# xenji/kafka-topic-analyzer

Measured on AMD Instinct MI355X. Metric: records/sec whole-node + achieved HBM GB/s, 256-part 256B-mean synthetic topic, higher is better.
Workload: dtype u64; 1 GPU; c4: 256-partition synthetic topic, mixed key/value sizes (mean record ~256 B), partitions sharded p % n_gpus; records_per_gpu=1073741824, partitions=256, partition_order=random, bytes_per_record=20, parallelism=partition-sharded x1, forced_collectives=False, exchange=none (1 GPU)

## Files before the change

### kafka_topic_analyzer_amd/csrc/kta_kernels.hip

```cpp
#include "kta_kernels.h"

#include <limits.h>
#include <type_traits>

namespace kta {


constexpr uint32_t kCntBits = 21;
constexpr uint64_t kCntMask = (1ull << kCntBits) - 1;
constexpr uint32_t kFlushTiles = 256;
#ifndef KTA_SCAN_PREFETCH
#define KTA_SCAN_PREFETCH 1
#endif
#ifndef KTA_PACKED_LOADS_ONLY
#define KTA_PACKED_LOADS_ONLY 0
#endif
constexpr int kTilePrefetch = KTA_SCAN_PREFETCH;
static_assert(kTilePrefetch == 1 || kTilePrefetch == 2, "the prefetch ring has two or three slots");
#ifndef KTA_PACKED_PREFETCH
#define KTA_PACKED_PREFETCH 1
#endif
constexpr int kPackedPrefetch = KTA_PACKED_PREFETCH;
static_assert(kPackedPrefetch == 1 || kPackedPrefetch == 2, "the prefetch ring has two or three slots");

struct Quad {
    int4 p, k, v;
    longlong2 t0, t1;
    long long base;
    uint32_t compact;
};
constexpr uint32_t kQuadCompact = 1u, kQuadLens16 = 2u, kQuadSummed = 4u;

typedef int v4i __attribute__((ext_vector_type(4)));
typedef int v2i __attribute__((ext_vector_type(2)));
typedef long long v2l __attribute__((ext_vector_type(2)));
static_assert(KTA_TILE_RECORDS == 4u * kWG, "a layout tile is one scan tile: 256 lanes x 4 records");

template <bool NT>
__device__ __forceinline__ void load_quad(Quad &q, const ScanColumns &c, uint64_t qi)
{
    if (NT) {
        const v4i p = __builtin_nontemporal_load(reinterpret_cast<const v4i *>(c.partition) + qi);
        const v4i k = __builtin_nontemporal_load(reinterpret_cast<const v4i *>(c.key_len) + qi);
        const v4i v = __builtin_nontemporal_load(reinterpret_cast<const v4i *>(c.val_len) + qi);
        const v2l t0 = __builtin_nontemporal_load(reinterpret_cast<const v2l *>(c.ts_ms) + 2 * qi);
        const v2l t1 = __builtin_nontemporal_load(reinterpret_cast<const v2l *>(c.ts_ms) + 2 * qi + 1);
        q.p = make_int4(p.x, p.y, p.z, p.w);
        q.k = make_int4(k.x, k.y, k.z, k.w);
        q.v = make_int4(v.x, v.y, v.z, v.w);
        q.t0 = make_longlong2(t0.x, t0.y);
        q.t1 = make_longlong2(t1.x, t1.y);
    } else {
        q.p = reinterpret_cast<const int4 *>(c.partition)[qi];
        q.k = reinterpret_cast<const int4 *>(c.key_len)[qi];
        q.v = reinterpret_cast<const int4 *>(c.val_len)[qi];
        q.t0 = reinterpret_cast<const longlong2 *>(c.ts_ms)[2 * qi];
        q.t1 = reinterpret_cast<const longlong2 *>(c.ts_ms)[2 * qi + 1];
    }
    q.compact = 0u;
}

template <bool NT>
__device__ __forceinline__ int4 load16(const void *col, uint64_t i)
{
    if (NT) {
        const v4i x = __builtin_nontemporal_load(reinterpret_cast<const v4i *>(col) + i);
        return make_int4(x.x, x.y, x.z, x.w);
    }
    return reinterpret_cast<const int4 *>(col)[i];
}

__device__ __forceinline__ void tile_sum_extrema(const kta_tile_hdr &h, const kta_tile_sum &s, long long &lo, long long &hi)
{
    const bool timed = (s.flags & KTA_TILE_SUM_TIMED) != 0, untimed = (s.flags & KTA_TILE_SUM_UNTIMED) != 0;
    lo = timed ? (long long)h.ts_base : LLONG_MAX;
    hi = timed ? (long long)((uint64_t)h.ts_base + s.ts_span) : LLONG_MIN;
    lo = (untimed && 0ll < lo) ? 0ll : lo;
    hi = (untimed && 0ll > hi) ? 0ll : hi;
}
__device__ __forceinline__ bool tile_summed(const kta_tile_hdr &h, const kta_tile_sum &s, uint64_t T, const ScanColumns &c, uint64_t n,
                                            uint32_t pc, long long &lo, long long &hi)
{
    const uint64_t first = T * KTA_TILE_RECORDS;
    if (!((s.flags & KTA_TILE_SUM_VALID) && first >= c.rec0 && first + KTA_TILE_RECORDS <= c.rec0 + n && s.part_max < pc)) return false;
    tile_sum_extrema(h, s, lo, hi);
    return true;
}

__device__ __forceinline__ uint32_t quad_valid(uint64_t a, uint64_t n)
{
    uint32_t valid = 0u;
#pragma unroll
    for (uint32_t j = 0; j < 4; j++) valid |= (a + j < n) ? 1u << j : 0u;
    return valid;
}

template <bool NT, bool SUM = false>
__device__ __forceinline__ void load_tile_quad(Quad &q, const ScanColumns &c, uint64_t T, uint32_t tid, uint64_t n = 0, uint32_t pc = 0)
{
    const kta_tile_hdr h = c.hdr[T];
    const kta_tile_sum sm = SUM ? c.sum[T] : kta_tile_sum{0, 0, 0};
    const uint64_t qi = T * (KTA_TILE_RECORDS / 4) + tid;
    const bool lens16 = h.lens == KTA_TILE_LENS_U16;
    q.k = load16<NT>(c.key_len, qi);
    if (!lens16) q.v = load16<NT>(c.val_len, qi);
    if (h.mode != KTA_TILE_COMPACT) {
        q.p = load16<NT>(c.partition, qi);
        const int4 a = load16<NT>(c.ts_ms, 2 * qi), b = load16<NT>(c.ts_ms, 2 * qi + 1);
        q.t0.x = (long long)(((uint64_t)(uint32_t)a.y << 32) | (uint32_t)a.x);
        q.t0.y = (long long)(((uint64_t)(uint32_t)a.w << 32) | (uint32_t)a.z);
        q.t1.x = (long long)(((uint64_t)(uint32_t)b.y << 32) | (uint32_t)b.x);
        q.t1.y = (long long)(((uint64_t)(uint32_t)b.w << 32) | (uint32_t)b.z);
        q.compact = lens16 ? kQuadLens16 : 0u;
        return;
    }
    const uint64_t ci = T * (KTA_TILE_RECORDS / 2) + tid;
    v2i p;
    if (NT) p = __builtin_nontemporal_load(reinterpret_cast<const v2i *>(c.partition) + ci);
    else p = reinterpret_cast<const v2i *>(c.partition)[ci];
    q.p.x = p.x;
    q.p.y = p.y;
    if (SUM) {
        long long lo, hi;
        if (tile_summed(h, sm, T, c, n, pc, lo, hi)) {
            q.t0.x = lo;
            q.t0.y = hi;
            q.compact = kQuadCompact | kQuadSummed | (lens16 ? kQuadLens16 : 0u);
            return;
        }
    }
    const int4 o = load16<NT>(c.ts_ms, ci);
    q.t0.x = (long long)(((uint64_t)(uint32_t)o.y << 32) | (uint32_t)o.x);
    q.t0.y = (long long)(((uint64_t)(uint32_t)o.w << 32) | (uint32_t)o.z);
    q.base = h.ts_base;
    q.compact = kQuadCompact | (lens16 ? kQuadLens16 : 0u);
}

__device__ __forceinline__ void quad_part_ts(const Quad &q, uint32_t (&p)[4], long long (&t)[4])
{
    if (q.compact & kQuadCompact) {
        uint32_t u[4];
        int32_t o[4];
        tile_u16x4((uint32_t)q.p.x, (uint32_t)q.p.y, u);
        tile_i32x4(q.t0.x, q.t0.y, o);
#pragma unroll
        for (int j = 0; j < 4; j++) {
            p[j] = (uint32_t)tile_unpack_part(u[j]);
            t[j] = tile_unpack_ts(o[j], q.base);
        }
    } else {
        p[0] = (uint32_t)q.p.x, p[1] = (uint32_t)q.p.y, p[2] = (uint32_t)q.p.z, p[3] = (uint32_t)q.p.w;
        t[0] = q.t0.x, t[1] = q.t0.y, t[2] = q.t1.x, t[3] = q.t1.y;
    }
// ... 473 lines not shown
constexpr uint32_t kFrontFlushTiles = 32;
constexpr uint64_t kFrontRecords = (uint64_t)kFrontFlushTiles * KTA_TILE_RECORDS;
static_assert(kFrontRecords <= 0xFFFFu, "count, tombstones and null keys of a front interval fit 16 bits");
static_assert(kFrontRecords + (kFrontRecords << 16) <= 0xFFFFFFFFull, "count | tombstones << 16 stays in W1's low dword");
static_assert(kFrontRecords * (KTA_COMPACT_LEN_NONE - 1u) < (1ull << 31), "a front interval's u16 sizes sum below 2^31");
static_assert(kFrontRecords * KTA_PLANE_KEY_NONE < (1ull << 23), "a front interval's raw plane key bytes sum below 2^23");
static_assert(kFrontRecords * KTA_COMPACT_LEN_NONE < (1ull << 31), "a front interval's raw plane value words sum below 2^31");

struct PackedLds {
    unsigned long long *W1, *W2;
    unsigned long long *B;
};

__device__ __forceinline__ unsigned long long pack_dwords(uint32_t lo, uint32_t hi)
{
    return ((unsigned long long)hi << 32) | lo;
}

template <bool LENS16>
__device__ __forceinline__ void packed_quad_lens(const Quad &q, const uint32_t (&pt)[4], const bool (&ok)[4], uint32_t P,
                                                 uint32_t rep_log2, uint32_t rep, const PackedLds &L, LaneState &st)
{
    uint32_t tomb[4], knull[4], ks[4], vs[4];
    if (LENS16) {
        uint32_t ku[4], vu[4];
        tile_u16x4((uint32_t)q.k.x, (uint32_t)q.k.y, ku);
        tile_u16x4((uint32_t)q.k.z, (uint32_t)q.k.w, vu);
#pragma unroll
        for (int j = 0; j < 4; j++) {
            knull[j] = ku[j] == KTA_COMPACT_LEN_NONE;
            tomb[j] = vu[j] == KTA_COMPACT_LEN_NONE;
            ks[j] = knull[j] ? 0u : ku[j];
            vs[j] = tomb[j] ? 0u : vu[j];
        }
    } else {
        const int32_t kl[4] = {q.k.x, q.k.y, q.k.z, q.k.w}, vl[4] = {q.v.x, q.v.y, q.v.z, q.v.w};
#pragma unroll
        for (int j = 0; j < 4; j++) {
            knull[j] = (uint32_t)kl[j] >> 31;
            tomb[j] = (uint32_t)vl[j] >> 31;
            ks[j] = knull[j] ? 0u : (uint32_t)kl[j];
            vs[j] = tomb[j] ? 0u : (uint32_t)vl[j];
        }
    }
#pragma unroll
    for (int j = 0; j < 4; j++) {
        const bool sized = ok[j] && !tomb[j];
        const uint32_t sz = ks[j] + vs[j];
        st.smin = min(st.smin, sized ? sz : 0xFFFFFFFFu);
        st.smax = max(st.smax, sized ? sz : 0u);
    }
#if KTA_PACKED_LOADS_ONLY
    st.bad += pt[0] ^ pt[1] ^ pt[2] ^ pt[3];
    return;
#endif
    const bool uniform = ok[0] && ok[1] && ok[2] && ok[3] && pt[0] == pt[1] && pt[0] == pt[2] && pt[0] == pt[3];
    if (uniform) {
        const uint32_t slot = (pt[0] << rep_log2) | rep;
        const uint32_t tombs = tomb[0] + tomb[1] + tomb[2] + tomb[3];
        const uint32_t knulls = knull[0] + knull[1] + knull[2] + knull[3];
        if (LENS16) {
            atomicAdd(&L.W1[slot], pack_dwords(4u | (tombs << 16), ks[0] + ks[1] + ks[2] + ks[3]));
            atomicAdd(&L.W2[slot], pack_dwords(knulls, vs[0] + vs[1] + vs[2] + vs[3]));
        } else {
            atomicAdd(&L.W1[slot], (unsigned long long)(4u | (tombs << 16)));
            atomicAdd(&L.W2[slot], (unsigned long long)knulls);
            atomicAdd(&L.B[3u * P + pt[0]], (unsigned long long)ks[0] + ks[1] + ks[2] + ks[3]);
            atomicAdd(&L.B[4u * P + pt[0]], (unsigned long long)vs[0] + vs[1] + vs[2] + vs[3]);
        }
        return;
    }
#pragma unroll
    for (int j = 0; j < 4; j++) {
        if (!ok[j]) continue;
        const uint32_t slot = (pt[j] << rep_log2) | rep;
        if (LENS16) {
            atomicAdd(&L.W1[slot], pack_dwords(1u | (tomb[j] << 16), ks[j]));
            atomicAdd(&L.W2[slot], pack_dwords(knull[j], vs[j]));
        } else {
            atomicAdd(&L.W1[slot], (unsigned long long)(1u | (tomb[j] << 16)));
            atomicAdd(&L.W2[slot], (unsigned long long)knull[j]);
            atomicAdd(&L.B[3u * P + pt[j]], (unsigned long long)ks[j]);
            atomicAdd(&L.B[4u * P + pt[j]], (unsigned long long)vs[j]);
        }
    }
}

template <int FORM, bool SUM>
__device__ __forceinline__ void packed_quad(const Quad &q, uint32_t valid, uint32_t P, uint32_t rep_log2, uint32_t rep,
                                            const PackedLds &L, LaneState &st)
{
    const uint32_t form = FORM >= 0 ? (uint32_t)FORM : q.compact;
    uint32_t pt[4];
    bool ok[4];
    if (SUM && (form & kQuadSummed)) {
        tile_u16x4((uint32_t)q.p.x, (uint32_t)q.p.y, pt);
#pragma unroll
        for (int j = 0; j < 4; j++) ok[j] = true;
        st.tmin = q.t0.x < st.tmin ? q.t0.x : st.tmin;
        st.tmax = q.t0.y > st.tmax ? q.t0.y : st.tmax;
    } else if (form & kQuadCompact) {
        static_assert(KTA_COMPACT_TS_NONE == INT32_MIN, "the sentinel is neutral for min as u32 and for max as i32");
        const uint32_t pc = min(P, (uint32_t)KTA_COMPACT_PART_NONE);
        int32_t o[4];
        tile_u16x4((uint32_t)q.p.x, (uint32_t)q.p.y, pt);
        tile_i32x4(q.t0.x, q.t0.y, o);
        uint32_t lo = (uint32_t)KTA_COMPACT_TS_NONE;
        int32_t hi = KTA_COMPACT_TS_NONE;
        bool none = false;
#pragma unroll
        for (int j = 0; j < 4; j++) {
            ok[j] = ((valid >> j) & 1u) && pt[j] < pc;
            const int32_t oj = ok[j] ? o[j] : KTA_COMPACT_TS_NONE;
            lo = min(lo, (uint32_t)oj);
            hi = max(hi, oj);
            none = none || (ok[j] && o[j] == KTA_COMPACT_TS_NONE);
        }
        const bool timed = hi >= 0;
        const long long tlo = (long long)((uint64_t)q.base + lo), thi = (long long)((uint64_t)q.base + (uint32_t)hi);
        st.tmin = (timed && tlo < st.tmin) ? tlo : st.tmin;
        st.tmax = (timed && thi > st.tmax) ? thi : st.tmax;
        st.tmin = (none && 0ll < st.tmin) ? 0ll : st.tmin;
        st.tmax = (none && 0ll > st.tmax) ? 0ll : st.tmax;
    } else {
        const long long ts[4] = {q.t0.x, q.t0.y, q.t1.x, q.t1.y};
        pt[0] = (uint32_t)q.p.x, pt[1] = (uint32_t)q.p.y, pt[2] = (uint32_t)q.p.z, pt[3] = (uint32_t)q.p.w;
#pragma unroll
        for (int j = 0; j < 4; j++) {
            ok[j] = ((valid >> j) & 1u) && pt[j] < P;
            const long long t = (ts[j] == -1ll) ? 0ll : ts[j];
            st.tmin = (ok[j] && t < st.tmin) ? t : st.tmin;
            st.tmax = (ok[j] && t > st.tmax) ? t : st.tmax;
        }
    }
    if (!(SUM && (form & kQuadSummed))) {
#pragma unroll
        for (int j = 0; j < 4; j++) st.bad += (((valid >> j) & 1u) && !ok[j]) ? 1u : 0u;
    }
    if (form & kQuadLens16) packed_quad_lens<true>(q, pt, ok, P, rep_log2, rep, L, st);
    else packed_quad_lens<false>(q, pt, ok, P, rep_log2, rep, L, st);
}

template <bool SUM>
__device__ __forceinline__ void accumulate_packed(const Quad &q, uint32_t valid, uint32_t P, uint32_t rep_log2, uint32_t rep,
                                                  const PackedLds &L, LaneState &st)
{
    constexpr uint32_t both = kQuadCompact | kQuadLens16, summed = both | kQuadSummed;
    if (SUM && q.compact == summed) packed_quad<(int)summed, SUM>(q, valid, P, rep_log2, rep, L, st);
    else if ((q.compact & both) == both) packed_quad<(int)both, SUM>(q, valid, P, rep_log2, rep, L, st);
    else packed_quad<-1, SUM>(q, valid, P, rep_log2, rep, L, st);
}

#ifndef KTA_LEAN_PREFETCH
#define KTA_LEAN_PREFETCH 1
#endif
constexpr int kLeanPrefetch = KTA_LEAN_PREFETCH;
static_assert(kLeanPrefetch >= 1 && kLeanPrefetch <= 3, "the lean ring has two, three or four slots");

struct LeanSlot {
    v2i p;
    int4 k;
};
struct PlaneSlot {
    int4 w;
};
constexpr uint64_t kTileColBytes = (uint64_t)KTA_TILE_RECORDS * 4u;

__device__ __forceinline__ void lean_tile(const kta_tile_hdr &h, const kta_tile_sum &s, uint32_t mark, bool whole, uint32_t pc,
                                          bool &lean, bool &plane)
{
    const bool summed = whole && (s.flags & KTA_TILE_SUM_VALID) && s.part_max < pc && h.mode == KTA_TILE_COMPACT;
    plane = summed && mark == 1u;
    lean = summed && !plane && h.lens == KTA_TILE_LENS_U16;
}

template <bool NT>
__device__ __forceinline__ void lean_load(LeanSlot &s, const ScanColumns &c, uint64_t T, uint32_t off8, uint32_t off16)
{
    const char *pb = reinterpret_cast<const char *>(c.partition) + T * kTileColBytes;
    const char *kb = reinterpret_cast<const char *>(c.key_len) + T * kTileColBytes;
    const v2i *pp = reinterpret_cast<const v2i *>(pb + off8);
    const v4i *kp = reinterpret_cast<const v4i *>(kb + off16);
    s.p = NT ? __builtin_nontemporal_load(pp) : *pp;
    const v4i k = NT ? __builtin_nontemporal_load(kp) : *kp;
    s.k = make_int4(k.x, k.y, k.z, k.w);
}
template <bool NT>
__device__ __forceinline__ void lean_load(PlaneSlot &s, const ScanColumns &c, uint64_t T, uint32_t, uint32_t off16)
{
    const char *tb = reinterpret_cast<const char *>(c.ts_ms) + T * (2u * kTileColBytes) + kTilePlaneOffset;
    const v4i *wp = reinterpret_cast<const v4i *>(tb + off16);
    const v4i w = NT ? __builtin_nontemporal_load(wp) : *wp;
    s.w = make_int4(w.x, w.y, w.z, w.w);
}

__device__ __forceinline__ void lean_quad_add(const uint32_t (&pt)[4], const uint32_t (&ku)[4], const uint32_t (&vu)[4],
                                              const uint32_t (&knull)[4], const uint32_t (&tomb)[4], uint32_t rep_log2, uint32_t rep,
                                              const PackedLds &L, LaneState &st)
{
    uint32_t ks[4], vs[4];
#pragma unroll
    for (int j = 0; j < 4; j++) {
        ks[j] = knull[j] ? 0u : ku[j];
        vs[j] = tomb[j] ? 0u : vu[j];
    }
    uint32_t lo[4], hi[4];
#pragma unroll
    for (int j = 0; j < 4; j++) {
        const uint32_t sz = ks[j] + vs[j];
        lo[j] = tomb[j] ? 0xFFFFFFFFu : sz;
        hi[j] = tomb[j] ? 0u : sz;
    }
    st.smin = min(min(min(lo[0], lo[1]), min(lo[2], lo[3])), st.smin);
    st.smax = max(max(max(hi[0], hi[1]), max(hi[2], hi[3])), st.smax);
#if KTA_PACKED_LOADS_ONLY
    st.bad += pt[0] ^ pt[1] ^ pt[2] ^ pt[3];
    return;
#endif
    if (pt[0] == pt[1] && pt[0] == pt[2] && pt[0] == pt[3]) {
        const uint32_t slot = (pt[0] << rep_log2) | rep;
        const uint32_t tombs = tomb[0] + tomb[1] + tomb[2] + tomb[3];
        const uint32_t knulls = knull[0] + knull[1] + knull[2] + knull[3];
        atomicAdd(&L.W1[slot], pack_dwords(4u | (tombs << 16), ks[0] + ks[1] + ks[2] + ks[3]));
        atomicAdd(&L.W2[slot], pack_dwords(knulls, vs[0] + vs[1] + vs[2] + vs[3]));
        return;
    }
#pragma unroll
    for (int j = 0; j < 4; j++) {
        const uint32_t slot = (pt[j] << rep_log2) | rep;
        atomicAdd(&L.W1[slot], pack_dwords(1u | (tomb[j] << 16), ks[j]));
        atomicAdd(&L.W2[slot], pack_dwords(knull[j], vs[j]));
    }
}
__device__ __forceinline__ void lean_quad(const LeanSlot &s, uint32_t rep_log2, uint32_t rep, const PackedLds &L, LaneState &st)
{
    uint32_t pt[4], ku[4], vu[4], tomb[4], knull[4];
    tile_u16x4((uint32_t)s.p.x, (uint32_t)s.p.y, pt);
    tile_u16x4((uint32_t)s.k.x, (uint32_t)s.k.y, ku);
    tile_u16x4((uint32_t)s.k.z, (uint32_t)s.k.w, vu);
#pragma unroll
    for (int j = 0; j < 4; j++) {
        knull[j] = ku[j] == KTA_COMPACT_LEN_NONE;
        tomb[j] = vu[j] == KTA_COMPACT_LEN_NONE;
    }
    lean_quad_add(pt, ku, vu, knull, tomb, rep_log2, rep, L, st);
}
__device__ __forceinline__ void lean_quad(const PlaneSlot &s, uint32_t rep_log2, uint32_t rep, const PackedLds &L, LaneState &st)
{
    const uint32_t w[4] = {(uint32_t)s.w.x, (uint32_t)s.w.y, (uint32_t)s.w.z, (uint32_t)s.w.w};
#if KTA_PACKED_LOADS_ONLY
    st.bad += w[0] ^ w[1] ^ w[2] ^ w[3];
    return;
#endif
    uint32_t pt[4], ku[4], vu[4], tomb[4], knull[4];
#pragma unroll
    for (int j = 0; j < 4; j++) {
        pt[j] = w[j] & 0xFFu;
        ku[j] = (w[j] >> 8) & 0xFFu;
        vu[j] = w[j] >> 16;
        knull[j] = ku[j] == KTA_PLANE_KEY_NONE;
        tomb[j] = vu[j] == KTA_COMPACT_LEN_NONE;
    }
    if (pt[0] == pt[1] && pt[0] == pt[2] && pt[0] == pt[3]) {
        const uint32_t slot = (pt[0] << rep_log2) | rep;
        const uint32_t tombs = tomb[0] + tomb[1] + tomb[2] + tomb[3];
        const uint32_t knulls = knull[0] + knull[1] + knull[2] + knull[3];
        atomicAdd(&L.W1[slot], pack_dwords(4u | (tombs << 16), ku[0] + ku[1] + ku[2] + ku[3]));
        atomicAdd(&L.W2[slot], pack_dwords(knulls, vu[0] + vu[1] + vu[2] + vu[3]));
        return;
    }
#pragma unroll
    for (int j = 0; j < 4; j++) {
        const uint32_t slot = (pt[j] << rep_log2) | rep;
        atomicAdd(&L.W1[slot], pack_dwords(1u | (tomb[j] << 16), ku[j]));
        atomicAdd(&L.W2[slot], pack_dwords(knull[j], vu[j]));
    }
}

struct PackedWg {
    PackedLds L;
    uint32_t P, rep_log2, rep, tid;
    LaneState st;

    __device__ __forceinline__ PackedWg(unsigned long long *lds, uint32_t P_, uint32_t rep_log2_) : P(P_), rep_log2(rep_log2_)
    {
        tid = threadIdx.x;
        const uint32_t slots = P << rep_log2;
        L = PackedLds{lds, lds + slots, lds + 2 * slots};
        for (uint32_t i = tid; i < 2 * slots + kScanCols * P; i += kWG) lds[i] = 0ull;
        __syncthreads();
        rep = tid & ((1u << rep_log2) - 1u);
    }
    __device__ __forceinline__ void front_flush(bool raw = false) const
    {
        const unsigned long long key_none = raw ? KTA_PLANE_KEY_NONE : 0u, val_none = raw ? KTA_COMPACT_LEN_NONE : 0u;
        __syncthreads();
        for (uint32_t p = tid; p < P; p += kWG) {
            unsigned long long w1 = 0, w2 = 0;
            for (uint32_t r = 0; r < (1u << rep_log2); r++) {
                const uint32_t s = (p << rep_log2) | r;
                w1 += L.W1[s];
                w2 += L.W2[s];
                L.W1[s] = 0ull;
                L.W2[s] = 0ull;
            }
            L.B[p] += w1 & 0xFFFFull;
            L.B[P + p] += (w1 >> 16) & 0xFFFFull;
            L.B[2u * P + p] += w2 & 0xFFFFFFFFull;
            L.B[3u * P + p] += (w1 >> 32) - key_none * (w2 & 0xFFFFFFFFull);
            L.B[4u * P + p] += (w2 >> 32) - val_none * ((w1 >> 16) & 0xFFFFull);
        }
        __syncthreads();
    }
    template <bool MERGE = false>
    __device__ __forceinline__ void write_row(uint64_t *row, long long (&s_red)[kWG / 64][6]) const
    {
        for (uint32_t p = tid; p < P; p += kWG)
#pragma unroll
            for (uint32_t j = 0; j < kScanCols; j++) {
                uint64_t &o = row[(uint64_t)p * kScanCols + j];
                if (MERGE) o += L.B[j * P + p];
                else o = L.B[j * P + p];
            }
        write_scan_globals<MERGE>(st, s_red, row, P, tid);
    }
};

constexpr uint32_t kLeanListed = 4;
constexpr uint32_t kScanListA = 5, kScanHandover = 6, kScanListB = 7;
__device__ __forceinline__ uint32_t lean_list_entry(uint64_t list_a, uint64_t list_b, uint32_t i)
{
    return (uint32_t)((i < 2 ? list_a : list_b) >> (32u * (i & 1u)));
}

struct LeanRun {
    uint32_t tile = 0;
    uint32_t step = 0;
    uint32_t end = 0;
    uint32_t whole_lo = 0, whole_hi = 0;
    uint32_t listed = 0;
    uint64_t list_a = 0, list_b = 0;
    uint32_t handover = 0;
    uint32_t since_flush = 0;
};

template <bool NT, bool PLANE>
__device__ __forceinline__ void lean_run(PackedWg &wg, LeanRun &r, const ScanColumns &c, uint64_t t0, uint32_t last, uint32_t pc,
                                         uint32_t rep_log2)
{
    using Slot = typename std::conditional<PLANE, PlaneSlot, LeanSlot>::type;
    const uint32_t tid = wg.tid;
    const uint32_t G = gridDim.x;
    uint32_t stop = r.end;
    bool switched = false;
    uint32_t issued = r.tile;
    uint32_t istep = r.step;
    uint32_t sw_step = 0;
    kta_tile_hdr ah;
    uint2 as;
    uint32_t am = 0;
    auto look_ahead = [&]() {
        const uint64_t T = t0 + (issued < last ? issued : last);
        ah = c.hdr[T], as = reinterpret_cast<const uint2 *>(c.sum)[T];
        if (c.mark) am = c.mark[T];
    };
    auto issue = [&](Slot &s, bool &v) {
        const uint64_t T = t0 + (issued < last ? issued : last);
        const bool in = issued < stop;
        const kta_tile_sum sm{as.x, (uint16_t)(as.y & 0xFFFFu), (uint16_t)(as.y >> 16)};
        bool lean, plane;
        lean_tile(ah, sm, am, issued >= r.whole_lo && issued < r.whole_hi, pc, lean, plane);
        v = (PLANE ? plane : lean) && in;
        const bool other = (PLANE ? lean : plane) && in;
        lean_load<NT>(s, c, T, 8u * tid, 16u * tid);
        if (other) {
            switched = true;
            sw_step = istep;
            stop = issued;
        } else if (in && !v) {
            if (r.listed == kLeanListed) {
                r.handover = istep + 1u;
                r.end = stop = issued;
            } else {
                const uint64_t e = (uint64_t)(istep + 1u) << (32u * (r.listed & 1u));
                if (r.listed < 2) r.list_a |= e;
                else r.list_b |= e;
                r.listed++;
            }
        }
        issued += G;
        istep++;
        look_ahead();
    };
    auto take = [&](const Slot &s, bool v) {
        if (v) {
            lean_quad(s, rep_log2, wg.rep, wg.L, wg.st);
            if (++r.since_flush == kFrontFlushTiles) {
                wg.front_flush(PLANE);
                r.since_flush = 0;
            }
        }
        r.tile += G;
    };
    Slot s0, s1, s2, s3;
    bool v0 = false, v1 = false, v2 = false, v3 = false;
    look_ahead();
    issue(s0, v0);
    if (kLeanPrefetch >= 2) issue(s1, v1);
    if (kLeanPrefetch == 3) issue(s2, v2);
    while (r.tile < stop) {
        if (kLeanPrefetch == 3) {
            issue(s3, v3);
            take(s0, v0);
            issue(s0, v0);
            take(s1, v1);
            issue(s1, v1);
            take(s2, v2);
            issue(s2, v2);
            take(s3, v3);
        } else if (kLeanPrefetch == 2) {
            issue(s2, v2);
            take(s0, v0);
            issue(s0, v0);
            take(s1, v1);
            issue(s1, v1);
            take(s2, v2);
        } else {
            issue(s1, v1);
            take(s0, v0);
            issue(s0, v0);
            take(s1, v1);
        }
    }
    r.step = istep - (uint32_t)kLeanPrefetch;
    if (switched) r.tile = blockIdx.x + sw_step * G, r.step = sw_step;
}

template <bool NT>
__device__ __forceinline__ void packed_scan_lean(const ScanColumns &c, uint64_t n, uint32_t P, uint32_t rep_log2,
                                                 uint64_t *__restrict__ partials, uint32_t row_len, unsigned long long *lds,
                                                 long long (&s_red)[kWG / 64][6])
{
    PackedWg wg(lds, P, rep_log2);
    const uint32_t tid = wg.tid;
    const uint64_t t0 = c.rec0 / KTA_TILE_RECORDS;
    const uint64_t ntiles = (c.rec0 + n + KTA_TILE_RECORDS - 1) / KTA_TILE_RECORDS - t0;
    const uint32_t pc = min(P, (uint32_t)KTA_COMPACT_PART_NONE);
    LeanRun r;
    r.tile = blockIdx.x;
    r.end = (uint32_t)ntiles;
    r.whole_lo = c.rec0 % KTA_TILE_RECORDS ? 1u : 0u;
    r.whole_hi = (uint32_t)((c.rec0 + n) / KTA_TILE_RECORDS - t0);
    const uint32_t last = r.end - 1u;
    bool plane = c.mark != nullptr;
    while (r.tile < r.end) {
        if (plane) lean_run<NT, true>(wg, r, c, t0, last, pc, rep_log2);
        else lean_run<NT, false>(wg, r, c, t0, last, pc, rep_log2);
        if (r.since_flush) {
            wg.front_flush(plane);
            r.since_flush = 0;
        }
        plane = !plane;
    }
    for (uint64_t i = blockIdx.x + (uint64_t)tid * gridDim.x; i < r.end; i += (uint64_t)kWG * gridDim.x) {
        const kta_tile_hdr h = c.hdr[t0 + i];
        const kta_tile_sum sm = c.sum[t0 + i];
        const uint32_t mark = c.mark ? c.mark[t0 + i] : 0u;
        bool lean, plane;
        lean_tile(h, sm, mark, i >= r.whole_lo && i < r.whole_hi, pc, lean, plane);
        long long lo, hi;
        tile_sum_extrema(h, sm, lo, hi);
        wg.st.tmin = ((lean || plane) && lo < wg.st.tmin) ? lo : wg.st.tmin;
        wg.st.tmax = ((lean || plane) && hi > wg.st.tmax) ? hi : wg.st.tmax;
        if (plane) {
            wg.st.smin = min(wg.st.smin, c.size[2 * (t0 + i)]);
            wg.st.smax = max(wg.st.smax, c.size[2 * (t0 + i) + 1]);
        }
    }
    uint64_t *row = partials + (uint64_t)blockIdx.x * row_len;
    wg.write_row(row, s_red);
    if (tid == 0) {
        uint64_t *g = row + (uint64_t)P * kScanCols;
        g[kScanListA] = r.list_a;
        g[kScanHandover] = r.handover;
        g[kScanListB] = r.list_b;
    }
}

template <bool NT, bool SUM>
__global__ __launch_bounds__(kWG) void kta_metrics_scan_packed(ScanColumns c, uint64_t n, uint32_t P, uint32_t rep_log2,
                                                               uint64_t *__restrict__ partials, uint32_t row_len)
{
    extern __shared__ unsigned long long lds[];
    __shared__ long long s_red[kWG / 64][6];

    if constexpr (SUM) {
        packed_scan_lean<NT>(c, n, P, rep_log2, partials, row_len, lds, s_red);
        return;
    }
    PackedWg wg(lds, P, rep_log2);
    const uint32_t tid = wg.tid;
    const uint64_t t0 = c.rec0 / KTA_TILE_RECORDS;
    const uint64_t ntiles = (c.rec0 + n + KTA_TILE_RECORDS - 1) / KTA_TILE_RECORDS - t0;
    uint32_t since_flush = 0;
    uint64_t tile = blockIdx.x;
    const uint32_t pc = min(P, (uint32_t)KTA_COMPACT_PART_NONE);
    Quad cur, nxt, nx2;
    if (tile < ntiles) load_tile_quad<NT, SUM>(cur, c, t0 + tile, tid, n, pc);
    if (kPackedPrefetch == 2 && tile + gridDim.x < ntiles) load_tile_quad<NT, SUM>(nxt, c, t0 + tile + gridDim.x, tid, n, pc);
    while (tile < ntiles) {
        const uint64_t ntile = tile + gridDim.x;
        const uint64_t ahead = tile + (uint64_t)kPackedPrefetch * gridDim.x;
        if (ahead < ntiles) load_tile_quad<NT, SUM>(kPackedPrefetch == 2 ? nx2 : nxt, c, t0 + ahead, tid, n, pc);

        const uint64_t a = (t0 + tile) * KTA_TILE_RECORDS + 4u * tid - c.rec0;
        const uint32_t valid = quad_valid(a, n);
        accumulate_packed<SUM>(cur, valid, P, rep_log2, wg.rep, wg.L, wg.st);

        if (++since_flush == kFrontFlushTiles) {
            wg.front_flush();
            since_flush = 0;
        }
        cur = nxt;
        if (kPackedPrefetch == 2) nxt = nx2;
        tile = ntile;
    }
    wg.front_flush();
    wg.write_row(partials + (uint64_t)blockIdx.x * row_len, s_red);
}

template <bool NT>
__global__ __launch_bounds__(kWG) void kta_metrics_scan_packed_rest(ScanColumns c, uint64_t n, uint32_t P, uint32_t rep_log2,
                                                                    uint64_t *__restrict__ partials, uint32_t row_len)
{
    extern __shared__ unsigned long long lds[];
    __shared__ long long s_red[kWG / 64][6];

    uint64_t *row = partials + (uint64_t)blockIdx.x * row_len;
    uint64_t *g = row + (uint64_t)P * kScanCols;
    const uint64_t list_a = g[kScanListA], list_b = g[kScanListB], handover = g[kScanHandover];
    if ((list_a | list_b | handover) == 0) return;

    PackedWg wg(lds, P, rep_log2);
    const uint32_t tid = wg.tid;
    const uint64_t t0 = c.rec0 / KTA_TILE_RECORDS;
    const uint64_t ntiles = (c.rec0 + n + KTA_TILE_RECORDS - 1) / KTA_TILE_RECORDS - t0;
    const uint32_t pc = min(P, (uint32_t)KTA_COMPACT_PART_NONE);
    uint32_t since_flush = 0;
    Quad cur, nxt;
    uint64_t first = handover;
    uint32_t nlist = 0;
    for (uint32_t li = 0; li < kLeanListed; li++) nlist += lean_list_entry(list_a, list_b, li) != 0u;
    while (first > 1 && nlist > 0 && lean_list_entry(list_a, list_b, nlist - 1u) == (uint32_t)(first - 1)) {
        first--;
        nlist--;
    }
    for (uint32_t li = 0; li < nlist; li++) {
        const uint64_t tile = blockIdx.x + (uint64_t)(lean_list_entry(list_a, list_b, li) - 1u) * gridDim.x;
        load_tile_quad<NT, false>(cur, c, t0 + tile, tid, n, pc);
        const uint64_t a = (t0 + tile) * KTA_TILE_RECORDS + 4u * tid - c.rec0;
        const uint32_t valid = quad_valid(a, n);
        accumulate_packed<false>(cur, valid, P, rep_log2, wg.rep, wg.L, wg.st);
        since_flush++;
    }
    uint64_t tile = first ? blockIdx.x + (first - 1) * gridDim.x : ntiles;
    if (tile < ntiles) load_tile_quad<NT, false>(cur, c, t0 + tile, tid, n, pc);
    while (tile < ntiles) {
        const uint64_t ntile = tile + gridDim.x;
        if (ntile < ntiles) load_tile_quad<NT, false>(nxt, c, t0 + ntile, tid, n, pc);

        const uint64_t a = (t0 + tile) * KTA_TILE_RECORDS + 4u * tid - c.rec0;
        const uint32_t valid = quad_valid(a, n);
        accumulate_packed<false>(cur, valid, P, rep_log2, wg.rep, wg.L, wg.st);

        if (++since_flush == kFrontFlushTiles) {
            wg.front_flush();
            since_flush = 0;
        }
        cur = nxt;
        tile = ntile;
    }
    wg.front_flush();
    wg.write_row<true>(row, s_red);
}

__global__ __launch_bounds__(kWG) void kta_fold_partials(const uint64_t *__restrict__ partials,
                                                         uint32_t rows, uint32_t P,
                                                         uint64_t *__restrict__ vec, uint32_t row_len,
                                                         uint64_t *__restrict__ avec)
{
    const uint32_t base_len = P * kScanCols + kScanGlobals;
    const uint32_t col = blockIdx.x * kWG + threadIdx.x;
    if (col >= row_len) return;
    const uint32_t r0 = (uint32_t)(((uint64_t)rows * blockIdx.y) / gridDim.y);
    const uint32_t r1 = (uint32_t)(((uint64_t)rows * (blockIdx.y + 1)) / gridDim.y);
    if (r0 == r1) return;
    if (col >= base_len) {
        const uint32_t a = col - base_len;
        if (a < 4u * P) {
            long long m = LLONG_MIN;
            for (uint32_t r = r0; r < r1; r++) {
                const long long x = (long long)partials[(uint64_t)r * row_len + col];
                m = x > m ? x : m;
            }
            atomicMax(reinterpret_cast<long long *>(avec) + 2 * kHistBuckets + a, m);
        } else {
            unsigned long long t = 0;
            for (uint32_t r = r0; r < r1; r++) t += partials[(uint64_t)r * row_len + col];
            if (t) atomicAdd(reinterpret_cast<unsigned long long *>(avec) + (a - 4u * P), t);
        }
        return;
    }
    unsigned long long *v = reinterpret_cast<unsigned long long *>(vec);
    unsigned long long *g = v + (uint64_t)P * 7;
    if (col < P * kScanCols) {
        const uint32_t p = col / kScanCols, f = col % kScanCols;
        unsigned long long s = 0;
        for (uint32_t r = r0; r < r1; r++) s += partials[(uint64_t)r * row_len + col];
        if (s == 0) return;
        unsigned long long *o = v + (uint64_t)p * 7;
        switch (f) {
        case 0:
            atomicAdd(&o[0], s);
            atomicAdd(&o[2], s);
            atomicAdd(&o[4], s);
            atomicAdd(&g[2], s);
            break;
        case 1:
            atomicAdd(&o[1], s);
            atomicAdd(&o[2], 0ull - s);
            break;
        case 2:
            atomicAdd(&o[3], s);
            atomicAdd(&o[4], 0ull - s);
            break;
        case 3: atomicAdd(&o[5], s); break;
        default: atomicAdd(&o[6], s); break;
        }
    } else {
        const uint32_t gi = col - P * kScanCols;
        long long *gs = reinterpret_cast<long long *>(g);
        if (gi == SG_TMIN || gi == SG_SMIN) {
            long long m = LLONG_MAX;
            for (uint32_t r = r0; r < r1; r++) {
                const long long x = (long long)partials[(uint64_t)r * row_len + col];
                m = x < m ? x : m;
            }
            atomicMax(&gs[gi == SG_TMIN ? 4 : 6], ~m);
        } else if (gi == SG_TMAX || gi == SG_SMAX) {
            long long m = LLONG_MIN;
            for (uint32_t r = r0; r < r1; r++) {
                const long long x = (long long)partials[(uint64_t)r * row_len + col];
                m = x > m ? x : m;
            }
            atomicMax(&gs[gi == SG_TMAX ? 5 : 7], m);
        } else if (gi == SG_BAD) {
            unsigned long long s = 0;
            for (uint32_t r = r0; r < r1; r++) s += partials[(uint64_t)r * row_len + col];
            if (s) atomicAdd(&g[0], s);
        }
    }
}

__global__ __launch_bounds__(kWG) void kta_tiles_to_raw(int32_t *__restrict__ partition, int64_t *__restrict__ ts_ms,
                                                        int32_t *__restrict__ key_len, int32_t *__restrict__ val_len,
                                                        kta_tile_hdr *__restrict__ hdr, uint64_t lo, uint64_t hi,
                                                        uint32_t what, uint32_t keep)
{
    const uint64_t t0 = lo / KTA_TILE_RECORDS, t1 = (hi + KTA_TILE_RECORDS - 1) / KTA_TILE_RECORDS;
    const uint32_t tid = threadIdx.x;
    for (uint64_t T = t0 + blockIdx.x; T < t1; T += gridDim.x) {
        const kta_tile_hdr h = hdr[T];
        const bool dm = (what & 1u) && h.mode == KTA_TILE_COMPACT, dl = (what & 2u) && h.lens == KTA_TILE_LENS_U16;
        if (!dm && !dl) continue;
        const uint64_t first = T * KTA_TILE_RECORDS;
        if (keep || first < lo || first + KTA_TILE_RECORDS > hi) {
            int32_t p[4];
            long long t[4];
            int4 g = make_int4(0, 0, 0, 0);
            if (dm) {
#pragma unroll
                for (uint32_t j = 0; j < 4; j++) tile_record_h<false>(partition, ts_ms, h, T, first + 4u * tid + j, p[j], t[j]);
// ... 165 lines not shown
```

Before: 1225 billion records/s.

## Classify lean tiles in 64-step wave ballots and stream by byte offset

Replaces the per-tile serial header lookahead in the lean scan with block classification: each lane of a wave loads one tile's header, summary, mark and size side data for a 64-step block, and ballots produce plane/lean masks that drive unrolled four-tile bodies. The trailing per-thread pass that recomputed timestamp and size extrema is folded into block opening. Tile addresses are now advanced by a precomputed byte stride. The lean prefetch depth is raised and the lean kernel gets a waves-per-SIMD launch bound, trading register budget for occupancy and adding control-flow complexity around partial blocks and handover.

```diff
diff --git a/kafka_topic_analyzer_amd/csrc/kta_kernels.hip b/kafka_topic_analyzer_amd/csrc/kta_kernels.hip
--- a/kafka_topic_analyzer_amd/csrc/kta_kernels.hip
+++ b/kafka_topic_analyzer_amd/csrc/kta_kernels.hip
@@ -1,4 +1,5 @@
 #include "kta_kernels.h"
+#include "kta_lean_blocks.h"
 
 #include <limits.h>
 #include <type_traits>
@@ -778,7 +779,7 @@
 }
 
 #ifndef KTA_LEAN_PREFETCH
-#define KTA_LEAN_PREFETCH 1
+#define KTA_LEAN_PREFETCH 2
 #endif
 constexpr int kLeanPrefetch = KTA_LEAN_PREFETCH;
 static_assert(kLeanPrefetch >= 1 && kLeanPrefetch <= 3, "the lean ring has two, three or four slots");
@@ -801,10 +802,10 @@
 }
 
 template <bool NT>
-__device__ __forceinline__ void lean_load(LeanSlot &s, const ScanColumns &c, uint64_t T, uint32_t off8, uint32_t off16)
-{
-    const char *pb = reinterpret_cast<const char *>(c.partition) + T * kTileColBytes;
-    const char *kb = reinterpret_cast<const char *>(c.key_len) + T * kTileColBytes;
+__device__ __forceinline__ void lean_load(LeanSlot &s, const ScanColumns &c, uint64_t B, uint32_t off8, uint32_t off16)
+{
+    const char *pb = reinterpret_cast<const char *>(c.partition) + B;
+    const char *kb = reinterpret_cast<const char *>(c.key_len) + B;
     const v2i *pp = reinterpret_cast<const v2i *>(pb + off8);
     const v4i *kp = reinterpret_cast<const v4i *>(kb + off16);
     s.p = NT ? __builtin_nontemporal_load(pp) : *pp;
@@ -812,9 +813,9 @@
     s.k = make_int4(k.x, k.y, k.z, k.w);
 }
 template <bool NT>
-__device__ __forceinline__ void lean_load(PlaneSlot &s, const ScanColumns &c, uint64_t T, uint32_t, uint32_t off16)
-{
-    const char *tb = reinterpret_cast<const char *>(c.ts_ms) + T * (2u * kTileColBytes) + kTilePlaneOffset;
+__device__ __forceinline__ void lean_load(PlaneSlot &s, const ScanColumns &c, uint64_t B, uint32_t, uint32_t off16)
+{
+    const char *tb = reinterpret_cast<const char *>(c.ts_ms) + B;
     const v4i *wp = reinterpret_cast<const v4i *>(tb + off16);
     const v4i w = NT ? __builtin_nontemporal_load(wp) : *wp;
     s.w = make_int4(w.x, w.y, w.z, w.w);
@@ -959,15 +960,30 @@
     return (uint32_t)((i < 2 ? list_a : list_b) >> (32u * (i & 1u)));
 }
 
+struct LeanSide {
+    kta_tile_hdr h;
+    uint2 s;
+    uint32_t m, z0, z1;
+};
+__device__ __forceinline__ void lean_side_load(LeanSide &sd, const ScanColumns &c, uint64_t T)
+{
+    const uint32_t *mp = c.mark ? c.mark : reinterpret_cast<const uint32_t *>(c.sum);
+    const uint32_t *zp = c.mark ? c.size : reinterpret_cast<const uint32_t *>(c.sum);
+    sd.h = c.hdr[T];
+    sd.s = reinterpret_cast<const uint2 *>(c.sum)[T];
+    sd.m = mp[T];
+    sd.z0 = zp[2u * T];
+    sd.z1 = zp[2u * T + 1u];
+}
+
 struct LeanRun {
-    uint32_t tile = 0;
+    LeanBlocks b;
     uint32_t step = 0;
-    uint32_t end = 0;
+    uint32_t open_at = 0;
+    uint64_t pm = 0, lm = 0;
     uint32_t whole_lo = 0, whole_hi = 0;
-    uint32_t listed = 0;
-    uint64_t list_a = 0, list_b = 0;
-    uint32_t handover = 0;
     uint32_t since_flush = 0;
+    LeanSide side;
 };
 
 template <bool NT, bool PLANE>
@@ -975,48 +991,23 @@
                                          uint32_t rep_log2)
 {
     using Slot = typename std::conditional<PLANE, PlaneSlot, LeanSlot>::type;
-    const uint32_t tid = wg.tid;
+    constexpr uint64_t kUnit = PLANE ? 2u * kTileColBytes : kTileColBytes;
+    const uint32_t tid = wg.tid, lane = tid & 63u;
     const uint32_t G = gridDim.x;
-    uint32_t stop = r.end;
-    bool switched = false;
-    uint32_t issued = r.tile;
-    uint32_t istep = r.step;
-    uint32_t sw_step = 0;
-    kta_tile_hdr ah;
-    uint2 as;
-    uint32_t am = 0;
-    auto look_ahead = [&]() {
-        const uint64_t T = t0 + (issued < last ? issued : last);
-        ah = c.hdr[T], as = reinterpret_cast<const uint2 *>(c.sum)[T];
-        if (c.mark) am = c.mark[T];
+    const uint64_t stride = (uint64_t)G * kUnit;
+    uint32_t itile = 0;
+    uint64_t ibyte = 0;
+    auto seek = [&](uint32_t step) {
+        const uint64_t tile = blockIdx.x + (uint64_t)step * G;
+        itile = tile < last ? (uint32_t)tile : last;
+        ibyte = (t0 + itile) * kUnit + (PLANE ? kTilePlaneOffset : 0u);
     };
-    auto issue = [&](Slot &s, bool &v) {
-        const uint64_t T = t0 + (issued < last ? issued : last);
-        const bool in = issued < stop;
-        const kta_tile_sum sm{as.x, (uint16_t)(as.y & 0xFFFFu), (uint16_t)(as.y >> 16)};
-        bool lean, plane;
-        lean_tile(ah, sm, am, issued >= r.whole_lo && issued < r.whole_hi, pc, lean, plane);
-        v = (PLANE ? plane : lean) && in;
-        const bool other = (PLANE ? lean : plane) && in;
-        lean_load<NT>(s, c, T, 8u * tid, 16u * tid);
-        if (other) {
-            switched = true;
-            sw_step = istep;
-            stop = issued;
-        } else if (in && !v) {
-            if (r.listed == kLeanListed) {
-                r.handover = istep + 1u;
-                r.end = stop = issued;
-            } else {
-                const uint64_t e = (uint64_t)(istep + 1u) << (32u * (r.listed & 1u));
-                if (r.listed < 2) r.list_a |= e;
-                else r.list_b |= e;
-                r.listed++;
-            }
-        }
-        issued += G;
-        istep++;
-        look_ahead();
+    auto issue = [&](Slot &s) {
+        lean_load<NT>(s, c, ibyte, 8u * tid, 16u * tid);
+        const uint32_t next = itile + G;
+        const bool adv = next <= last;
+        itile = adv ? next : itile;
+        ibyte += adv ? stride : 0ull;
     };
     auto take = [&](const Slot &s, bool v) {
         if (v) {
@@ -1026,40 +1017,95 @@
                 r.since_flush = 0;
             }
         }
-        r.tile += G;
     };
-    Slot s0, s1, s2, s3;
-    bool v0 = false, v1 = false, v2 = false, v3 = false;
-    look_ahead();
-    issue(s0, v0);
-    if (kLeanPrefetch >= 2) issue(s1, v1);
-    if (kLeanPrefetch == 3) issue(s2, v2);
-    while (r.tile < stop) {
+    auto side_request = [&](uint32_t base) {
+        const uint64_t tile = blockIdx.x + (uint64_t)(base + lane) * G;
+        lean_side_load(r.side, c, t0 + (tile < last ? tile : last));
+    };
+    auto open_block = [&]() {
+        const uint32_t base = r.open_at;
+        const uint64_t tile = blockIdx.x + (uint64_t)(base + lane) * G;
+        const kta_tile_sum sm{r.side.s.x, (uint16_t)(r.side.s.y & 0xFFFFu), (uint16_t)(r.side.s.y >> 16)};
+        bool lean, plane;
+        lean_tile(r.side.h, sm, c.mark ? r.side.m : 0u, tile >= r.whole_lo && tile < r.whole_hi, pc, lean, plane);
+        r.pm = __ballot(plane);
+        r.lm = __ballot(lean);
+        lean_block(r.b, base, kLeanListed, r.pm, r.lm);
+        const bool tp = (r.pm >> lane) & 1ull, tl = (r.lm >> lane) & 1ull;
+        long long lo, hi;
+        tile_sum_extrema(r.side.h, sm, lo, hi);
+        wg.st.tmin = ((tp || tl) && lo < wg.st.tmin) ? lo : wg.st.tmin;
+        wg.st.tmax = ((tp || tl) && hi > wg.st.tmax) ? hi : wg.st.tmax;
+        wg.st.smin = min(wg.st.smin, tp ? r.side.z0 : 0xFFFFFFFFu);
+        wg.st.smax = max(wg.st.smax, tp ? r.side.z1 : 0u);
+        r.open_at = base + kLeanBlockSteps;
+        side_request(r.open_at);
+    };
+    auto span = [&](uint64_t &mine) {
+        const uint32_t pos = r.step - (r.open_at - kLeanBlockSteps);
+        const uint64_t a = (PLANE ? r.pm : r.lm) >> pos, o = (PLANE ? r.lm : r.pm) >> pos;
+        uint32_t cnt = o ? (uint32_t)__builtin_ctzll(o) : kLeanBlockSteps - pos;
+        cnt = min(cnt, r.b.end - r.step);
+        mine = cnt < kLeanBlockSteps ? a & ((1ull << cnt) - 1ull) : a;
+        return cnt;
+    };
+    Slot a, b, cc, d;
+    auto body = [&](uint64_t &m) {
         if (kLeanPrefetch == 3) {
-            issue(s3, v3);
-            take(s0, v0);
-            issue(s0, v0);
-            take(s1, v1);
-            issue(s1, v1);
-            take(s2, v2);
-            issue(s2, v2);
-            take(s3, v3);
+            issue(d), take(a, (uint32_t)m & 1u);
+            issue(a), take(b, (uint32_t)m & 2u);
+            issue(b), take(cc, (uint32_t)m & 4u);
+            issue(cc), take(d, (uint32_t)m & 8u);
         } else if (kLeanPrefetch == 2) {
-            issue(s2, v2);
-            take(s0, v0);
-            issue(s0, v0);
-            take(s1, v1);
-            issue(s1, v1);
-            take(s2, v2);
+            issue(cc), take(a, (uint32_t)m & 1u);
+            issue(d), take(b, (uint32_t)m & 2u);
+            issue(a), take(cc, (uint32_t)m & 4u);
+            issue(b), take(d, (uint32_t)m & 8u);
         } else {
-            issue(s1, v1);
-            take(s0, v0);
-            issue(s0, v0);
-            take(s1, v1);
-        }
-    }
-    r.step = istep - (uint32_t)kLeanPrefetch;
-    if (switched) r.tile = blockIdx.x + sw_step * G, r.step = sw_step;
+            issue(b), take(a, (uint32_t)m & 1u);
+            issue(a), take(b, (uint32_t)m & 2u);
+            issue(b), take(a, (uint32_t)m & 4u);
+            issue(a), take(b, (uint32_t)m & 8u);
+        }
+        m >>= 4;
+    };
+    if (r.step != r.open_at) {
+        uint64_t mine;
+        uint32_t cnt = span(mine);
+        const bool ends = cnt < r.open_at - r.step;
+        while ((r.step & 3u) && cnt) {
+            Slot x;
+            seek(r.step);
+            issue(x);
+            take(x, mine & 1u);
+            mine >>= 1;
+            r.step++, cnt--;
+        }
+        if (!cnt && ends) return;
+    }
+    seek(r.step);
+    issue(a);
+    if (kLeanPrefetch >= 2) issue(b);
+    if (kLeanPrefetch == 3) issue(cc);
+    while (r.step < r.b.end) {
+        uint64_t mine;
+        uint32_t cnt, nb;
+        const bool opens = r.step == r.open_at;
+        if (opens) {
+            open_block();
+            cnt = span(mine);
+            if (!cnt) break;
+            nb = (cnt + 3u) / 4u - 1u;
+            body(mine);
+        } else {
+            cnt = span(mine);
+            if (!cnt) break;
+            nb = (cnt + 3u) / 4u;
+        }
+        for (; nb; nb--) body(mine);
+        r.step += cnt;
+        if (r.step != r.open_at) break;
+    }
 }
 
 template <bool NT>
@@ -1073,13 +1119,16 @@
     const uint64_t ntiles = (c.rec0 + n + KTA_TILE_RECORDS - 1) / KTA_TILE_RECORDS - t0;
     const uint32_t pc = min(P, (uint32_t)KTA_COMPACT_PART_NONE);
     LeanRun r;
-    r.tile = blockIdx.x;
-    r.end = (uint32_t)ntiles;
+    r.b.end = lean_steps(blockIdx.x, gridDim.x, ntiles);
     r.whole_lo = c.rec0 % KTA_TILE_RECORDS ? 1u : 0u;
     r.whole_hi = (uint32_t)((c.rec0 + n) / KTA_TILE_RECORDS - t0);
-    const uint32_t last = r.end - 1u;
+    const uint32_t last = (uint32_t)ntiles - 1u;
     bool plane = c.mark != nullptr;
-    while (r.tile < r.end) {
+    if (r.b.end) {
+        const uint64_t tile = blockIdx.x + (uint64_t)(tid & 63u) * gridDim.x;
+        lean_side_load(r.side, c, t0 + (tile < last ? tile : last));
+    }
+    while (r.step < r.b.end) {
         if (plane) lean_run<NT, true>(wg, r, c, t0, last, pc, rep_log2);
         else lean_run<NT, false>(wg, r, c, t0, last, pc, rep_log2);
         if (r.since_flush) {
@@ -1088,28 +1137,13 @@
         }
         plane = !plane;
     }
-    for (uint64_t i = blockIdx.x + (uint64_t)tid * gridDim.x; i < r.end; i += (uint64_t)kWG * gridDim.x) {
-        const kta_tile_hdr h = c.hdr[t0 + i];
-        const kta_tile_sum sm = c.sum[t0 + i];
-        const uint32_t mark = c.mark ? c.mark[t0 + i] : 0u;
-        bool lean, plane;
-        lean_tile(h, sm, mark, i >= r.whole_lo && i < r.whole_hi, pc, lean, plane);
-        long long lo, hi;
-        tile_sum_extrema(h, sm, lo, hi);
-        wg.st.tmin = ((lean || plane) && lo < wg.st.tmin) ? lo : wg.st.tmin;
-        wg.st.tmax = ((lean || plane) && hi > wg.st.tmax) ? hi : wg.st.tmax;
-        if (plane) {
-            wg.st.smin = min(wg.st.smin, c.size[2 * (t0 + i)]);
-            wg.st.smax = max(wg.st.smax, c.size[2 * (t0 + i) + 1]);
-        }
-    }
     uint64_t *row = partials + (uint64_t)blockIdx.x * row_len;
     wg.write_row(row, s_red);
     if (tid == 0) {
         uint64_t *g = row + (uint64_t)P * kScanCols;
-        g[kScanListA] = r.list_a;
-        g[kScanHandover] = r.handover;
-        g[kScanListB] = r.list_b;
+        g[kScanListA] = r.b.list_a;
+        g[kScanHandover] = r.b.handover;
+        g[kScanListB] = r.b.list_b;
     }
 }
 
@@ -1154,6 +1188,22 @@
     wg.front_flush();
     wg.write_row(partials + (uint64_t)blockIdx.x * row_len, s_red);
 }
+#ifndef KTA_LEAN_WAVES
+#define KTA_LEAN_WAVES 5
+#endif
+constexpr int kLeanWavesPerSimd = KTA_LEAN_WAVES;
+#define KTA_LEAN_KERNEL(NT)                                                                                                    \
+    template <>                                                                                                                \
+    __global__ __launch_bounds__(kWG, kLeanWavesPerSimd) void kta_metrics_scan_packed<NT, true>(                               \
+        ScanColumns c, uint64_t n, uint32_t P, uint32_t rep_log2, uint64_t *__restrict__ partials, uint32_t row_len)           \
+    {                                                                                                                          \
+        extern __shared__ unsigned long long lds[];                                                                            \
+        __shared__ long long s_red[kWG / 64][6];                                                                               \
+        packed_scan_lean<NT>(c, n, P, rep_log2, partials, row_len, lds, s_red);                                                \
+    }
+KTA_LEAN_KERNEL(true)
+KTA_LEAN_KERNEL(false)
+#undef KTA_LEAN_KERNEL
 
 template <bool NT>
 __global__ __launch_bounds__(kWG) void kta_metrics_scan_packed_rest(ScanColumns c, uint64_t n, uint32_t P, uint32_t rep_log2,
diff --git a/kafka_topic_analyzer_amd/csrc/kta_lean_blocks.h b/kafka_topic_analyzer_amd/csrc/kta_lean_blocks.h
--- /dev/null
+++ b/kafka_topic_analyzer_amd/csrc/kta_lean_blocks.h
@@ -0,0 +1,53 @@
+#pragma once
+
+#include <stdint.h>
+
+#ifdef __HIPCC__
+#define KTA_LEAN_HD __host__ __device__
+#else
+#define KTA_LEAN_HD
+#endif
+
+namespace kta {
+
+constexpr uint32_t kLeanBlockSteps = 64;
+
+struct LeanBlocks {
+    uint32_t end = 0;
+    uint32_t listed = 0;
+    uint64_t list_a = 0, list_b = 0;
+    uint32_t handover = 0;
+};
+
+KTA_LEAN_HD inline uint32_t lean_steps(uint32_t wg, uint32_t grid, uint64_t ntiles)
+{
+    return wg < ntiles ? (uint32_t)((ntiles - 1u - wg) / grid) + 1u : 0u;
+}
+
+KTA_LEAN_HD inline void lean_block(LeanBlocks &s, uint32_t base, uint32_t max_listed, uint64_t &plane, uint64_t &lean)
+{
+    const uint32_t left = s.end > base ? s.end - base : 0u;
+    const uint64_t in = left >= kLeanBlockSteps ? ~0ull : (1ull << left) - 1ull;
+    plane &= in;
+    lean &= in & ~plane;
+    uint64_t others = in & ~(plane | lean);
+    while (others) {
+        const uint32_t l = (uint32_t)__builtin_ctzll(others);
+        others &= others - 1ull;
+        const uint32_t step = base + l;
+        if (s.listed == max_listed) {
+            const uint64_t before = (1ull << l) - 1ull;
+            s.handover = step + 1u;
+            s.end = step;
+            plane &= before;
+            lean &= before;
+            return;
+        }
+        const uint64_t e = (uint64_t)(step + 1u) << (32u * (s.listed & 1u));
+        if (s.listed < 2) s.list_a |= e;
+        else s.list_b |= e;
+        s.listed++;
+    }
+}
+
+}
```

Measured after the change: 1299 billion records/s (median of 6 runs). 6.0% higher.
